# apachepinot/pinot

Measured on AMD Instinct MI355X. Metric: rows scanned/sec, 1B-row segment filter+groupby (3 predicates, SUM/MAX GROUP BY g1), higher is better.
Workload: dtype int64; 1 GPU; 1 segment(s) x 1000000000 rows, one per GPU; SELECT g1, SUM(m), MAX(m) FROM gpuBench WHERE c_inv1 IN (0,1,2,3) AND c_inv2 IN (0,1) AND r_int BETWEEN 250000 AND 749999 GROUP BY g1 ORDER BY g1 LIMIT 1000; query=cfg3, parallelism=segment-per-gpu x1, merge=none (1 segment), entries_scanned_in_filter=249990290

## Files before the change

pinot_amd/csrc/pg_kernels_spec.hip:

```cpp
#define PG_WAVES_PER_BLOCK 12
#define PG_KERNEL template <int PG_NOT_INSTANTIATED> static
#include "pg_kernels.hip"

#define SPEC_LOADERS 4
#ifndef SPEC_TILES
#define SPEC_TILES 2
#endif
#ifndef SPEC_SETS
#define SPEC_SETS 2
#endif
#define SPEC_CONSUMERS 8
#define SPEC_OFF_LIN 0u
#define SPEC_OFF_RNG 256u
#define SPEC_OFF_VAL (256u + 2048u)
#define SPEC_OFF_G0 (256u + 2048u + 8192u)
extern "C" const int pg_spec_waves_per_block = PG_WAVES_PER_BLOCK;
extern "C" int pg_spec_stage_bytes(int bits0, int bits1) { return SPEC_TILES * (((int)SPEC_OFF_G0 + bits0 * 256 + 16 + (bits1 > 0 ? bits1 * 256 + 16 : 0) + 15) & ~15); }

DEVFN void spec_barrier() {
  __builtin_amdgcn_fence(__ATOMIC_RELEASE, "workgroup", "local");
  __builtin_amdgcn_s_barrier();
  __builtin_amdgcn_fence(__ATOMIC_ACQUIRE, "workgroup", "local");
}

template <typename T> DEVFN const GAS T* spec_sgpr_ptr(const void* ptr) {
  const uint64_t v = (uint64_t)ptr;
  const uint32_t lo = (uint32_t)__builtin_amdgcn_readfirstlane((int)(uint32_t)v), hi = (uint32_t)__builtin_amdgcn_readfirstlane((int)(uint32_t)(v >> 32));
  return (const GAS T*)(((uint64_t)hi << 32) | (uint64_t)lo);
}

template <int W> struct SpecCol;
template <> struct SpecCol<0> {};
template <> struct SpecCol<32> { u32x4 r[2]; };
template <> struct SpecCol<24> { u32x4 lo; u32x2 hi; };
template <> struct SpecCol<16> { u32x4 lo; };
template <> struct SpecCol<8> { u32x2 hi; };
constexpr uint32_t spec_img_tile_bytes(int W) { return (uint32_t)(PG_WAVE_DOCS / 8) * (uint32_t)W; }
template <int W> DEVFN void spec_load(SpecCol<W>& c, const uint8_t* base, int wt, int w, int lane) {
  if constexpr (W == 32) {
#pragma unroll
    for (int s = 0; s < 2; s++) {
      const uint8_t* row = base + (size_t)wt * (PG_WAVE_DOCS * 4) + (size_t)(4 * s + w) * 1024u;
      c.r[s] = ldnt((const GAS u32x4*)(spec_sgpr_ptr<uint8_t>(row) + (uint32_t)lane * 16u));
    }
  } else if constexpr (W != 0) {
    const uint8_t* tile = base + (size_t)wt * spec_img_tile_bytes(W);
    if constexpr (W >= 16) c.lo = ldnt((const GAS u32x4*)(spec_sgpr_ptr<uint8_t>(tile + (size_t)w * 1024u) + (uint32_t)lane * 16u));
    if constexpr (W != 16) c.hi = ldnt((const GAS u32x2*)(spec_sgpr_ptr<uint8_t>(tile + (W == 24 ? 4096u : 0u) + (size_t)w * 512u) + (uint32_t)lane * 8u));
  }
}
template <int W> DEVFN void spec_unpack(const SpecCol<W>& c, uint32_t (&a)[4], uint32_t (&b)[4]) {
  if constexpr (W == 32) {
    a[0] = bswap32(c.r[0].x); a[1] = bswap32(c.r[0].y); a[2] = bswap32(c.r[0].z); a[3] = bswap32(c.r[0].w);
    b[0] = bswap32(c.r[1].x); b[1] = bswap32(c.r[1].y); b[2] = bswap32(c.r[1].z); b[3] = bswap32(c.r[1].w);
  } else if constexpr (W == 24) {
    a[0] = __builtin_amdgcn_perm(c.hi.x, c.lo.x, 0x0c040100u); a[1] = __builtin_amdgcn_perm(c.hi.x, c.lo.x, 0x0c050302u);
    a[2] = __builtin_amdgcn_perm(c.hi.x, c.lo.y, 0x0c060100u); a[3] = __builtin_amdgcn_perm(c.hi.x, c.lo.y, 0x0c070302u);
    b[0] = __builtin_amdgcn_perm(c.hi.y, c.lo.z, 0x0c040100u); b[1] = __builtin_amdgcn_perm(c.hi.y, c.lo.z, 0x0c050302u);
    b[2] = __builtin_amdgcn_perm(c.hi.y, c.lo.w, 0x0c060100u); b[3] = __builtin_amdgcn_perm(c.hi.y, c.lo.w, 0x0c070302u);
  } else if constexpr (W == 16) {
    a[0] = c.lo.x & 0xFFFFu; a[1] = c.lo.x >> 16; a[2] = c.lo.y & 0xFFFFu; a[3] = c.lo.y >> 16;
    b[0] = c.lo.z & 0xFFFFu; b[1] = c.lo.z >> 16; b[2] = c.lo.w & 0xFFFFu; b[3] = c.lo.w >> 16;
  } else if constexpr (W == 8) {
#pragma unroll
    for (int e = 0; e < 4; e++) { a[e] = (c.hi.x >> (8 * e)) & 0xFFu; b[e] = (c.hi.y >> (8 * e)) & 0xFFu; }
  }
}
template <int SW, int VW> struct SpecTile {
  SpecCol<SW> scan;
  SpecCol<VW> val;
  u32x4 grp;
};
template <int SW, int VW> struct SpecStage { SpecTile<SW, VW> tile[SPEC_TILES]; uint32_t post[8]; uint32_t tail; };
template <int NG> struct SpecQuad {
  uint32_t lin, rng;
  u32x4 val;
  uint32_t win[NG][2];
};

template <int W> struct SpecWidth { static constexpr int value = W; };
template <int NG, bool HAS_INDEX, bool HAS_SCAN, bool HAS_TAIL = false, bool NARROW = false>
__device__ __forceinline__ void spec_body(const PgQueryPlan& p) {
  extern __shared__ __attribute__((aligned(16))) uint64_t smem[];
  __shared__ uint32_t s_stat[PG_MAX_STATS];
  const int t = threadIdx.x;
  const int lane = t & 63;
  const int wave = uniform(t >> 6);
  int64_t* lds_table = reinterpret_cast<int64_t*>(smem);
  if (t < PG_MAX_STATS) s_stat[t] = 0;
  const uint32_t real_slots = (uint32_t)p.n_groups * (uint32_t)p.replicas;
  const uint32_t table_slots = real_slots + 64u;
  for (int o = 0; o < p.n_ops; o++) {
    const int64_t ident = pg_acc_identity(p.ops[o].fn, p.ops[o].is_float);
    for (uint32_t i = t; i < table_slots; i += PG_BLOCK) lds_table[(size_t)o * table_slots + i] = ident;
  }
  const uint32_t bits0 = (uint32_t)p.gcols[0].bits, bits1 = NG > 1 ? (uint32_t)p.gcols[NG - 1].bits : 0u;
  const uint32_t off_g1 = SPEC_OFF_G0 + bits0 * 256u + 16u;
  const uint32_t tile_bytes = (off_g1 + (NG > 1 ? bits1 * 256u + 16u : 0u) + 15u) & ~15u;
  const uint32_t stage_bytes = tile_bytes * SPEC_TILES;
  uint8_t* stage0 = reinterpret_cast<uint8_t*>(smem) + (((size_t)p.n_ops * table_slots * 8u + 15u) & ~(size_t)15u);
  const CAS PgScanLeaf& L = cptr(p.scans)[HAS_SCAN ? p.fast_scan : 0];
  const int grid = (int)gridDim.x;
  const int n_mine = (int)blockIdx.x < p.n_wtiles ? (p.n_wtiles - (int)blockIdx.x + grid - 1) / grid : 0;
  const int n_stages = (n_mine + SPEC_TILES - 1) / SPEC_TILES;
  __syncthreads();

  if (wave < SPEC_LOADERS) {
    const int w = wave;
    const uint8_t* const xdata = p.srcs[p.pipe_src].data;
    const uint8_t* const simg = NARROW ? p.spec_simg : nullptr;
    const uint8_t* const vimg = NARROW ? p.spec_vimg : nullptr;
    const uint32_t img_slo = NARROW ? p.spec_slo : 0u, img_sspan = NARROW ? p.spec_sspan : 0u, img_vmin = NARROW ? (uint32_t)p.spec_vmin : 0u;
    const bool img_sempty = NARROW && p.spec_sempty != 0;
    const int ggi = (w >> 1) < NG ? (w >> 1) : 0;
    const uint8_t* const gdata = p.gcols[ggi].data;
    const uint32_t gbits = (uint32_t)p.gcols[ggi].bits;
    const uint32_t goff = (uint32_t)(w & 1) * 1024u + (uint32_t)lane * 16u;
    const uint32_t geff = (w >> 1) < NG && goff < gbits * 256u ? goff : 0u;
    const uint8_t* dense_ptr[8];
    int dense_group[8];
#pragma unroll
    for (int j = 0; j < 8; j++) { dense_ptr[j] = HAS_INDEX ? p.dense_ptr[j] : nullptr; dense_group[j] = HAS_INDEX ? p.dense_group[j] : 0; }
    const int dense_groups = p.dense_groups, dense_excl = p.dense_excl;
    const uint8_t* const pipe_tail = HAS_TAIL ? p.pipe_tail : nullptr;
    const int num_docs = p.num_docs;
    const bool scan_pushed = p.fast_scan_pushed != 0;
   auto loaders = [&](auto scan_w, auto val_w) __attribute__((always_inline)) {
    constexpr int SW = HAS_SCAN ? decltype(scan_w)::value : 0, VW = decltype(val_w)::value;
    const RangeI32 r32 = !HAS_SCAN ? RangeI32{0, 0u, false} : (SW == 32 ? make_range_i32(L.lo, L.hi) : RangeI32{(int32_t)img_slo, img_sspan, img_sempty});
    const uint8_t* sdata = !HAS_SCAN ? nullptr : (SW == 32 ? L.data : simg);
    const uint8_t* vdata = VW == 32 ? xdata : vimg;
    const uint32_t vmin = VW == 32 ? 0u : img_vmin;
    uint32_t ld_cand = 0;
    auto issue = [&](int sidx, SpecStage<SW, VW>& st) __attribute__((always_inline)) {
#pragma unroll
      for (int tt = 0; tt < SPEC_TILES; tt++) {
        const int i = sidx * SPEC_TILES + tt;
        const int wt = (int)blockIdx.x + (i < n_mine ? i : n_mine - 1) * grid;
        SpecTile<SW, VW>& tl = st.tile[tt];
        __builtin_amdgcn_sched_barrier(0);
        spec_load<SW>(tl.scan, sdata, wt, w, lane);
        spec_load<VW>(tl.val, vdata, wt, w, lane);
        __builtin_amdgcn_sched_barrier(0);
        {
          const uint8_t* base = gdata + (size_t)wt * (size_t)(PG_WAVE_DOCS / 8) * (size_t)gbits;
          tl.grp = ldnt((const GAS u32x4*)(spec_sgpr_ptr<uint8_t>(base) + geff));
        }
        __builtin_amdgcn_sched_barrier(0);
      }
      if (HAS_INDEX) {
        const int i = sidx * SPEC_TILES + (w % SPEC_TILES);
        const int wt = (int)blockIdx.x + (i < n_mine ? i : n_mine - 1) * grid;
#pragma unroll
        for (int j = 0; j < 8; j++) st.post[j] = *(const GAS uint32_t*)(spec_sgpr_ptr<uint8_t>(dense_ptr[j] + (size_t)wt * 256u) + (uint32_t)lane * 4u);
        __builtin_amdgcn_sched_barrier(0);
      }
      if (HAS_TAIL) {
        const int i = sidx * SPEC_TILES + (w % SPEC_TILES);
        const int wt = (int)blockIdx.x + (i < n_mine ? i : n_mine - 1) * grid;
        st.tail = *(const GAS uint32_t*)(spec_sgpr_ptr<uint8_t>(pipe_tail + (size_t)wt * 256u) + (uint32_t)lane * 4u);
        __builtin_amdgcn_sched_barrier(0);
      }
    };
    auto publish = [&](uint8_t* stage, const SpecStage<SW, VW>& st) __attribute__((always_inline)) {
#ifdef PG_SPEC_NO_PUBLISH
      {
        uint32_t acc = 0;
#pragma unroll
        for (int tt = 0; tt < SPEC_TILES; tt++) {
          uint32_t a[4] = {0u, 0u, 0u, 0u}, b[4] = {0u, 0u, 0u, 0u};
          spec_unpack<SW>(st.tile[tt].scan, a, b); acc += a[0] ^ b[3];
          spec_unpack<VW>(st.tile[tt].val, a, b); acc += a[0] ^ b[3];
          acc += st.tile[tt].grp.x;
        }
        if (acc == 0x12345678u) *reinterpret_cast<uint32_t*>(stage) = acc;
        return;
      }
#endif
#pragma unroll
      for (int tt = 0; tt < SPEC_TILES; tt++) {
        uint8_t* buf = stage + (uint32_t)tt * tile_bytes;
        const SpecTile<SW, VW>& tl = st.tile[tt];
        if (HAS_SCAN) {
          uint32_t q[2][4];
          spec_unpack<SW>(tl.scan, q[0], q[1]);
#pragma unroll
          for (int s = 0; s < 2; s++) {
            uint32_t m = (uint32_t)in_range_i32(r32, (int32_t)q[s][0]) | ((uint32_t)in_range_i32(r32, (int32_t)q[s][1]) << 1) |
                         ((uint32_t)in_range_i32(r32, (int32_t)q[s][2]) << 2) | ((uint32_t)in_range_i32(r32, (int32_t)q[s][3]) << 3);
            m = r32.empty ? 0u : m;
            *reinterpret_cast<uint32_t*>(buf + SPEC_OFF_RNG + (uint32_t)(4 * s + w) * 256u + (uint32_t)lane * 4u) = m;
          }
        }
        {
          uint32_t q[2][4];
          spec_unpack<VW>(tl.val, q[0], q[1]);
#pragma unroll
          for (int s = 0; s < 2; s++) {
            u32x4 v;
            v.x = q[s][0] + vmin; v.y = q[s][1] + vmin; v.z = q[s][2] + vmin; v.w = q[s][3] + vmin;
            *reinterpret_cast<u32x4*>(buf + SPEC_OFF_VAL + (uint32_t)(4 * s + w) * 1024u + (uint32_t)lane * 16u) = v;
          }
        }
        *reinterpret_cast<u32x4*>(buf + (ggi == 0 ? SPEC_OFF_G0 : off_g1) + geff) = tl.grp;
      }
    };
    auto publish_lin = [&](uint8_t* stage, const SpecStage<SW, VW>& st, int sidx) __attribute__((always_inline)) {
      if (w >= SPEC_TILES) return;
      const int i = sidx * SPEC_TILES + w;
      const int wt = (int)blockIdx.x + i * grid;
      const int64_t rem = i < n_mine ? (int64_t)num_docs - (int64_t)wt * PG_WAVE_DOCS : 0;
      const int32_t n_valid = rem >= PG_WAVE_DOCS ? PG_WAVE_DOCS : (rem > 0 ? (int32_t)rem : 0);
      uint32_t lin = valid_lin_mask(n_valid, lane);
      if (HAS_INDEX) {
        uint32_t grp[4] = {0u, 0u, 0u, 0u};
#pragma unroll
        for (int j = 0; j < 8; j++) {
          const int gj = dense_group[j];
#pragma unroll
          for (int k = 0; k < 4; k++) grp[k] |= gj == k ? st.post[j] : 0u;
        }
#pragma unroll
        for (int k = 0; k < 4; k++)
          if (k < dense_groups) lin &= ((dense_excl >> k) & 1) ? ~grp[k] : grp[k];
      }
      *reinterpret_cast<uint32_t*>(stage + (uint32_t)w * tile_bytes + SPEC_OFF_LIN + (uint32_t)lane * 4u) = HAS_TAIL ? lin & st.tail : lin;
      ld_cand += (uint32_t)__popc(lin);
    };
    constexpr int SETS = HAS_SCAN ? SPEC_SETS : 2 * SPEC_SETS;
    SpecStage<SW, VW> st[SETS];
    auto buf_of = [&](int sg) __attribute__((always_inline)) { return stage0 + (uint32_t)(sg & 1) * stage_bytes; };
    if (n_stages > 0) {
#pragma unroll
      for (int k = 0; k < SETS; k++) issue(k, st[k]);
    }
    int s = 0;
    for (; s + SETS - 1 < n_stages; s += SETS) {
#pragma unroll
      for (int k = 0; k < SETS; k++) {
        publish(buf_of(s + k), st[k]);
        publish_lin(buf_of(s + k), st[k], s + k);
        issue(s + k + SETS, st[k]);
        spec_barrier();
      }
    }
#pragma unroll
    for (int k = 0; k < SETS - 1; k++)
      if (s + k < n_stages) {
        publish(buf_of(s + k), st[k]);
        publish_lin(buf_of(s + k), st[k], s + k);
        spec_barrier();
      }
    const uint32_t csum = wave_sum_u32(ld_cand);
    if (HAS_SCAN && !scan_pushed && lane == 0 && csum) atomicAdd(&s_stat[L.stat_slot], csum);
   };
    if constexpr (!NARROW) {
      loaders(SpecWidth<32>{}, SpecWidth<32>{});
    } else {
      const int sb = uniform(p.spec_sbits), vb = uniform(p.spec_vbits);
      auto with_scan = [&](auto scan_w) __attribute__((always_inline)) {
        switch (vb) {
          case 8: loaders(scan_w, SpecWidth<8>{}); break;
          case 16: loaders(scan_w, SpecWidth<16>{}); break;
          case 24: loaders(scan_w, SpecWidth<24>{}); break;
          default: loaders(scan_w, SpecWidth<32>{}); break;
        }
      };
      switch (sb) {
        case 8: with_scan(SpecWidth<8>{}); break;
        case 16: with_scan(SpecWidth<16>{}); break;
        case 24: with_scan(SpecWidth<24>{}); break;
        default: with_scan(SpecWidth<32>{}); break;
      }
    }
  } else {
    const int c = wave - SPEC_LOADERS;
    const uint32_t R = (uint32_t)p.replicas;
    const uint32_t rep = (uint32_t)t & (R - 1u);
    const uint32_t stride = table_slots;
    const uint32_t trash_slot = real_slots + (uint32_t)lane;
    const uint32_t q = (uint32_t)c * 64u + (uint32_t)lane;
    const uint32_t nib = ((uint32_t)lane & 7u) * 4u;
    uint32_t my_matched = 0;
    const int n_ops = uniform(p.n_ops);
    uint64_t ops_code = 0;
    for (int o = 0; o < n_ops; o++) {
      const PgAccOp op = p.ops[uniform(o)];
      ops_code |= (uint64_t)(op.src < 0 ? 0u : (op.fn == PG_ACC_SUM ? 1u : (op.fn == PG_ACC_MIN ? 2u : 3u))) << (2 * o);
    }
    ops_code = ((uint64_t)(uint32_t)uniform((int)(uint32_t)(ops_code >> 32)) << 32) | (uint64_t)(uint32_t)uniform((int)(uint32_t)ops_code);
    const int has_out_words = uniform(p.out_words != nullptr ? 1 : 0);
    auto fetch = [&](const uint8_t* buf, SpecQuad<NG>& d) __attribute__((always_inline)) {
      d.lin = *reinterpret_cast<const uint32_t*>(buf + SPEC_OFF_LIN + (q >> 3) * 4u);
      d.rng = HAS_SCAN ? *reinterpret_cast<const uint32_t*>(buf + SPEC_OFF_RNG + q * 4u) : 0xFu;
      d.val = *reinterpret_cast<const u32x4*>(buf + SPEC_OFF_VAL + q * 16u);
#pragma unroll
      for (int gi = 0; gi < NG; gi++) {
        const uint32_t di = __umul24(4u * q, (uint32_t)p.gcols[gi].bits) >> 5;
        const uint32_t* win = reinterpret_cast<const uint32_t*>(buf + (gi == 0 ? SPEC_OFF_G0 : off_g1)) + di;
        d.win[gi][0] = win[0]; d.win[gi][1] = win[1];
      }
    };
    auto aggregate = [&](const SpecQuad<NG> (&d)[SPEC_TILES], int sidx) __attribute__((always_inline)) {
      constexpr int ND = 4 * SPEC_TILES;
      uint32_t slot[ND];
      int32_t v[ND];
#pragma unroll
      for (int tt = 0; tt < SPEC_TILES; tt++) {
        const int i = sidx * SPEC_TILES + tt;
        const uint32_t cand = (d[tt].lin >> nib) & 0xFu;
        const uint32_t m = d[tt].rng & cand;
        my_matched += (uint32_t)__popc(m);
        if (has_out_words && i < n_mine) {
          const int wt = (int)blockIdx.x + i * grid;
          const uint32_t word = or_reduce8(m << nib);
          if ((lane & 7) == 0) reinterpret_cast<uint32_t*>(p.out_words)[(int64_t)wt * 64 + (int64_t)(q >> 3)] = word;
        }
#ifndef PG_SPEC_NO_TABLE
#pragma unroll
        for (int e = 0; e < 4; e++) slot[4 * tt + e] = rep;
#pragma unroll
        for (int gi = 0; gi < NG; gi++) {
          const PgGroupCol& gc = p.gcols[gi];
          const uint32_t bits = (uint32_t)gc.bits, mask = (1u << gc.bits) - 1u;
          const uint32_t mult = (uint32_t)gc.mult * R;
          uint32_t dv[4];
          decode_packed_quad<true>(d[tt].win[gi], q, bits, mask, dv);
#pragma unroll
          for (int e = 0; e < 4; e++) slot[4 * tt + e] += __umul24(dv[e], mult);
        }
#pragma unroll
        for (int e = 0; e < 4; e++) slot[4 * tt + e] = ((m >> e) & 1u) ? slot[4 * tt + e] : trash_slot;
        v[4 * tt + 0] = (int32_t)d[tt].val.x; v[4 * tt + 1] = (int32_t)d[tt].val.y; v[4 * tt + 2] = (int32_t)d[tt].val.z; v[4 * tt + 3] = (int32_t)d[tt].val.w;
#endif
      }
#ifdef PG_SPEC_NO_TABLE
      return;
#endif
      for (int o = 0; o < n_ops; o++) {
        const uint32_t code = (uint32_t)(ops_code >> (2 * o)) & 3u;
        int64_t* base = lds_table + (size_t)o * stride;
        if (code == 0u) {
#pragma unroll
          for (int e = 0; e < ND; e++) atomicAdd(reinterpret_cast<unsigned long long*>(base + slot[e]), 1ULL);
        } else if (code == 1u) {
#pragma unroll
          for (int e = 0; e < ND; e++) atomicAdd(reinterpret_cast<unsigned long long*>(base + slot[e]), (unsigned long long)(int64_t)v[e]);
        } else if (code == 2u) {
#pragma unroll
          for (int e = 0; e < ND; e++) atomicMin(reinterpret_cast<long long*>(base + slot[e]), (long long)v[e]);
        } else {
#pragma unroll
          for (int e = 0; e < ND; e++) atomicMax(reinterpret_cast<long long*>(base + slot[e]), (long long)v[e]);
        }
      }
    };
    auto fetch_stage = [&](int sidx, SpecQuad<NG> (&d)[SPEC_TILES]) __attribute__((always_inline)) {
// ... 83 lines not shown
```

pinot_amd/csrc/pg_segment.cpp:

```cpp
#include <hip/hip_runtime.h>

#include <algorithm>
#include <cmath>

#include "pg_internal.hpp"

extern "C" __global__ void __launch_bounds__(256) pg_column_magnitude_kernel(const uint8_t* __restrict__ data, int64_t n, int val_type,
                                                                             unsigned long long* __restrict__ out) {
  unsigned long long mx = 0, bad = 0;
  for (int64_t i = (int64_t)blockIdx.x * blockDim.x + threadIdx.x; i < n; i += (int64_t)gridDim.x * blockDim.x) {
    unsigned long long a;
    if (val_type == PG_V_I64) {
      const unsigned long long v = __builtin_bswap64(reinterpret_cast<const unsigned long long*>(data)[i]);
      a = (long long)v < 0 ? 0ULL - v : v;
    } else {
      double d;
      if (val_type == PG_V_F32) d = (double)__uint_as_float(__builtin_bswap32(reinterpret_cast<const uint32_t*>(data)[i]));
      else d = __longlong_as_double((long long)__builtin_bswap64(reinterpret_cast<const unsigned long long*>(data)[i]));
      a = (unsigned long long)__double_as_longlong(d) & 0x7FFFFFFFFFFFFFFFULL;
      if (a >= 0x7FF0000000000000ULL) { bad = 1; a = 0; }
    }
    mx = a > mx ? a : mx;
  }
  for (int off = 32; off > 0; off >>= 1) {
    const unsigned long long o = __shfl_xor(mx, off, 64);
    mx = o > mx ? o : mx;
    bad |= __shfl_xor(bad, off, 64);
  }
  if ((threadIdx.x & 63) == 0) {
    if (mx) atomicMax(&out[0], mx);
    if (bad) atomicOr(&out[1], 1ULL);
  }
}

extern "C" __global__ void __launch_bounds__(256) pg_column_int_range_kernel(const uint8_t* __restrict__ data, int64_t n, int val_type,
                                                                             long long* __restrict__ out) {
  long long mn = INT64_MAX, mx = INT64_MIN;
  for (int64_t i = (int64_t)blockIdx.x * blockDim.x + threadIdx.x; i < n; i += (int64_t)gridDim.x * blockDim.x) {
    const long long v = val_type == PG_V_I64 ? (long long)__builtin_bswap64(reinterpret_cast<const unsigned long long*>(data)[i])
                                             : (long long)(int32_t)__builtin_bswap32(reinterpret_cast<const uint32_t*>(data)[i]);
    mn = v < mn ? v : mn;
    mx = v > mx ? v : mx;
  }
  for (int off = 32; off > 0; off >>= 1) {
    const long long a = __shfl_xor(mn, off, 64), b = __shfl_xor(mx, off, 64);
    mn = a < mn ? a : mn;
    mx = b > mx ? b : mx;
  }
  if ((threadIdx.x & 63) == 0 && mn <= mx) {
    atomicMin(&out[0], mn);
    atomicMax(&out[1], mx);
  }
}

extern "C" __global__ void __launch_bounds__(256) pg_column_narrow_image_kernel(const uint8_t* __restrict__ data, uint8_t* __restrict__ img,
                                                                                int64_t n_wtiles, int32_t vmin, int bits) {
  const int64_t n = n_wtiles * 256;
  const int64_t tile_bytes = (int64_t)(PG_WAVE_DOCS / 8) * bits;
  for (int64_t i = (int64_t)blockIdx.x * blockDim.x + threadIdx.x; i < n; i += (int64_t)gridDim.x * blockDim.x) {
    const int64_t wt = i >> 8;
    const int b = (int)(i >> 6) & 3, l = (int)i & 63;
    const uint4 qa = *reinterpret_cast<const uint4*>(data + wt * (PG_WAVE_DOCS * 4) + (int64_t)b * 1024 + l * 16);
    const uint4 qb = *reinterpret_cast<const uint4*>(data + wt * (PG_WAVE_DOCS * 4) + (int64_t)(4 + b) * 1024 + l * 16);
    const uint32_t raw[8] = {qa.x, qa.y, qa.z, qa.w, qb.x, qb.y, qb.z, qb.w};
    uint32_t s[8];
    for (int e = 0; e < 8; e++) s[e] = (__builtin_bswap32(raw[e]) - (uint32_t)vmin) & (bits == 24 ? 0xFFFFFFu : (bits == 16 ? 0xFFFFu : 0xFFu));
    uint8_t* tile = img + wt * tile_bytes;
    if (bits >= 16) {
      uint4 lo;
      lo.x = (s[0] & 0xFFFFu) | (s[1] << 16); lo.y = (s[2] & 0xFFFFu) | (s[3] << 16);
      lo.z = (s[4] & 0xFFFFu) | (s[5] << 16); lo.w = (s[6] & 0xFFFFu) | (s[7] << 16);
      *reinterpret_cast<uint4*>(tile + (int64_t)b * 1024 + l * 16) = lo;
    }
    if (bits != 16) {
      const int sh = bits == 24 ? 16 : 0;
      uint2 hi;
      hi.x = ((s[0] >> sh) & 0xFFu) | (((s[1] >> sh) & 0xFFu) << 8) | (((s[2] >> sh) & 0xFFu) << 16) | (((s[3] >> sh) & 0xFFu) << 24);
      hi.y = ((s[4] >> sh) & 0xFFu) | (((s[5] >> sh) & 0xFFu) << 8) | (((s[6] >> sh) & 0xFFu) << 16) | (((s[7] >> sh) & 0xFFu) << 24);
      *reinterpret_cast<uint2*>(tile + (bits == 24 ? 4096 : 0) + (int64_t)b * 512 + l * 8) = hi;
    }
  }
}

extern "C" __global__ void __launch_bounds__(256) pg_column_max_dict_id_kernel(const uint8_t* __restrict__ data, int64_t n, int bits,
                                                                                unsigned int* __restrict__ out) {
  unsigned int mx = 0;
  const uint64_t mask = (1ULL << bits) - 1ULL;
  for (int64_t i = (int64_t)blockIdx.x * blockDim.x + threadIdx.x; i < n; i += (int64_t)gridDim.x * blockDim.x) {
    const uint64_t bit = (uint64_t)i * (uint64_t)bits;
    const uint8_t* p = data + (bit >> 3);
    uint64_t w = 0;
    for (int k = 0; k < 8; k++) w = (w << 8) | p[k];
    const unsigned int v = (unsigned int)((w >> (64 - bits - (int)(bit & 7))) & mask);
    mx = v > mx ? v : mx;
  }
  for (int off = 32; off > 0; off >>= 1) {
    const unsigned int o = __shfl_xor(mx, off, 64);
    mx = o > mx ? o : mx;
  }
  if ((threadIdx.x & 63) == 0 && mx) atomicMax(out, mx);
}

namespace pg {

static int32_t fx_exp_of(double max_abs) {
  if (!(max_abs > 0)) return 0;
  int e = 0;
  (void)std::frexp(max_abs, &e);
  return (int32_t)(16 * (int)std::floor(((double)e + 15.0) / 16.0));
}

static inline uint32_t be32(const uint8_t* p) {
  return ((uint32_t)p[0] << 24) | ((uint32_t)p[1] << 16) | ((uint32_t)p[2] << 8) | (uint32_t)p[3];
}
static inline uint64_t be64(const uint8_t* p) { return ((uint64_t)be32(p) << 32) | be32(p + 4); }
static inline uint16_t le16(const uint8_t* p) { return (uint16_t)(p[0] | (p[1] << 8)); }
static inline uint32_t le32(const uint8_t* p) {
  return (uint32_t)p[0] | ((uint32_t)p[1] << 8) | ((uint32_t)p[2] << 16) | ((uint32_t)p[3] << 24);
}

Column* Segment::find(const char* n) {
  if (!n) return nullptr;
  auto it = columns.find(n);
  return it == columns.end() ? nullptr : it->second.get();
}

static size_t padded_docs(const Segment& seg) { return (size_t)seg.n_tiles * PG_TILE_DOCS; }

static void check_dict_ids(const Column& c, int64_t n) {
  if (n <= 0 || c.cardinality <= 0 || !(c.bits >= 31 || ((int64_t)1 << c.bits) > (int64_t)c.cardinality)) return;
  DeviceBuffer out(4, true);
  const int grid = (int)std::max<int64_t>(1, std::min<int64_t>(2048, (n + 255) / 256));
  hipLaunchKernelGGL(pg_column_max_dict_id_kernel, dim3(grid), dim3(256), 0, 0, c.fwd_dev.as<uint8_t>(), n, c.bits, out.as<unsigned int>());
  PG_HIP(hipGetLastError());
  unsigned int mx = 0;
  PG_HIP(hipMemcpy(&mx, out.ptr, 4, hipMemcpyDeviceToHost));
  if ((int64_t)mx >= (int64_t)c.cardinality)
    fail(PG_ERR_INVALID_ARGUMENT, "forward index of %s holds dictId %u, the dictionary has %d values", c.name.c_str(), mx, c.cardinality);
}

static void upload_fixed_bit(Segment& seg, Column& c, const uint8_t* src, uint64_t len) {
  uint64_t need = ((uint64_t)seg.total_docs * (uint64_t)c.bits + 7) / 8;
  if (len < need) fail(PG_ERR_INVALID_ARGUMENT, "forward index of %s is %llu bytes, need %llu", c.name.c_str(),
                       (unsigned long long)len, (unsigned long long)need);
  size_t alloc = (padded_docs(seg) * (size_t)c.bits + 7) / 8 + 64;
  c.fwd_dev.alloc(alloc, true);
  c.fwd_dev.upload(src, need);
  c.col_kind = PG_COL_FIXED_BIT;
  c.fwd_bytes_logical = need;
  check_dict_ids(c, (int64_t)seg.total_docs);
}

static void parse_inverted_index(Segment& seg, Column& c, const uint8_t* inv, uint64_t len) {
  const int32_t card = c.cardinality;
  const uint64_t off_end = ((uint64_t)card + 1) * 4;
  if (len < off_end) fail(PG_ERR_INVALID_ARGUMENT, "inverted index of %s too short", c.name.c_str());
  const uint64_t first = be32(inv);
  const uint8_t* bitmap_buffer = inv + off_end;
  c.posting_begin.assign((size_t)card + 1, 0);
  std::vector<uint8_t> staging;
  staging.reserve(len);
  const uint32_t max_key = (uint32_t)((padded_docs(seg) + PG_CHUNK_DOCS - 1) / PG_CHUNK_DOCS);
// ... 693 lines not shown
      offs.resize((size_t)used_chunks + 1);
      decompress_fixed_byte_chunks(compression, fwd, offs, (uint32_t)docs_per_chunk * (uint32_t)width, need, c.fwd_dev.as<uint8_t>(), d.name);
    }
    c.col_kind = width == 4 ? PG_COL_RAW32 : PG_COL_RAW64;
    c.fwd_bytes_logical = need;
  } else {
    fail(PG_ERR_UNSUPPORTED, "column %s: forward index encoding %d", d.name, c.fwd_encoding);
  }

  if (c.has_dictionary && (c.data_type == PG_TYPE_LONG || c.data_type == PG_TYPE_FLOAT || c.data_type == PG_TYPE_DOUBLE)) {
    const uint8_t* dp = c.dict_host.data();
    double mx = 0;
    for (int32_t i = 0; i < c.cardinality; i++) {
      if (c.data_type == PG_TYPE_LONG) {
        const int64_t v = (int64_t)be64(dp + (size_t)i * 8);
        const uint64_t a = v < 0 ? 0ULL - (uint64_t)v : (uint64_t)v;
        c.max_abs_int = std::max(c.max_abs_int, a);
      } else {
        double v;
        if (c.data_type == PG_TYPE_FLOAT) { uint32_t u = be32(dp + (size_t)i * 4); float f; memcpy(&f, &u, 4); v = (double)f; }
        else { uint64_t u = be64(dp + (size_t)i * 8); memcpy(&v, &u, 8); }
        if (std::isfinite(v)) mx = std::max(mx, std::fabs(v));
        else c.has_nonfinite = true;
      }
    }
    c.fx_exp = fx_exp_of(mx);
  } else if (!c.has_dictionary && (c.val_type == PG_V_I64 || c.val_type == PG_V_F32 || c.val_type == PG_V_F64) &&
             (c.col_kind == PG_COL_RAW32 || c.col_kind == PG_COL_RAW64) && seg.total_docs > 0) {
    DeviceBuffer out(16, true);
    hipLaunchKernelGGL(pg_column_magnitude_kernel, dim3(1024), dim3(256), 0, 0, c.fwd_dev.as<uint8_t>(), (int64_t)seg.total_docs, c.val_type,
                       out.as<unsigned long long>());
    PG_HIP(hipGetLastError());
    unsigned long long h[2] = {0, 0};
    PG_HIP(hipMemcpy(h, out.ptr, sizeof(h), hipMemcpyDeviceToHost));
    if (c.val_type == PG_V_I64) c.max_abs_int = h[0];
    else {
      double mx;
      memcpy(&mx, &h[0], 8);
      c.fx_exp = fx_exp_of(mx);
      c.has_nonfinite = h[1] != 0;
    }
  }

  if (!c.has_dictionary && (c.val_type == PG_V_I32 || c.val_type == PG_V_I64) && (c.col_kind == PG_COL_RAW32 || c.col_kind == PG_COL_RAW64) &&
      seg.total_docs > 0) {
    const long long init[2] = {INT64_MAX, INT64_MIN};
    DeviceBuffer out(16);
    out.upload(init, sizeof(init));
    hipLaunchKernelGGL(pg_column_int_range_kernel, dim3(1024), dim3(256), 0, 0, c.fwd_dev.as<uint8_t>(), (int64_t)seg.total_docs, c.val_type,
                       out.as<long long>());
    PG_HIP(hipGetLastError());
    long long h[2] = {0, 0};
    PG_HIP(hipMemcpy(h, out.ptr, sizeof(h), hipMemcpyDeviceToHost));
    if (h[0] <= h[1]) { c.has_int_range = true; c.int_min = h[0]; c.int_max = h[1]; }
  }

  if (d.inverted_index.size > 0 && c.has_dictionary && c.fwd_encoding != PG_FWD_DICT_SORTED)
    parse_inverted_index(seg, c, (const uint8_t*)d.inverted_index.addr, d.inverted_index.size);

  seg.device_bytes += c.fwd_dev.size + c.dict_dev.size + c.containers_dev.size + c.descs_dev.size + c.mv_offsets_dev.size + c.vb_offsets_dev.size;
  seg.columns.emplace(c.name, std::move(col));
}

bool narrow_image_eligible(const Column& c) {
  return !c.has_dictionary && !c.is_mv && !c.raw_mv && c.col_kind == PG_COL_RAW32 && c.val_type == PG_V_I32 && c.has_int_range &&
         c.int_max - c.int_min < ((int64_t)1 << 24);
}

bool narrow_image(Segment& seg, Column& c) {
  std::lock_guard<std::mutex> g(seg.mu);
  if (c.img_state != 0) return c.img_state == 1;
  c.img_state = 2;
  const int64_t n_wtiles = (int64_t)seg.n_tiles * PG_WTILES_PER_TILE;
  if (!narrow_image_eligible(c) || n_wtiles <= 0 || c.fwd_dev.size < (size_t)n_wtiles * (PG_WAVE_DOCS * 4)) return false;
  const int64_t span = c.int_max - c.int_min;
  const int bits = span < 256 ? 8 : (span < 65536 ? 16 : 24);
  void* ptr = nullptr;
  const size_t bytes = (size_t)(n_wtiles * narrow_image_tile_bytes(bits));
  if (hipMalloc(&ptr, bytes) != hipSuccess) {
    (void)hipGetLastError();
    return false;
  }
  c.img_dev.ptr = ptr; c.img_dev.size = bytes; c.img_dev.device = seg.device;
  const int grid = (int)std::min<int64_t>((n_wtiles * 256 + 255) / 256, 8192);
  hipLaunchKernelGGL(pg_column_narrow_image_kernel, dim3(grid), dim3(256), 0, 0, c.fwd_dev.as<uint8_t>(), c.img_dev.as<uint8_t>(), n_wtiles,
                     (int32_t)c.int_min, bits);
  PG_HIP(hipGetLastError());
  PG_HIP(hipDeviceSynchronize());
  c.img_bits = bits;
  c.img_state = 1;
  seg.device_bytes += bytes;
  return true;
}

}
```

Baseline: 820.7 billion rows/s.

## Assign each spec loader wave a half-tile with wider loads and split roles

Loader waves change from loading a quarter-row slice of both tiles in a stage to owning one half of a single tile (tile w>>1, half w&1). Each wave now issues wider contiguous loads: four 16-byte rows for 32-bit data, and 16-byte instead of 8-byte high-byte loads for narrow data. It also loads every group column itself, and only the half-0 waves fetch the index postings and tail. The narrow-image layout and the kernel that builds it are rearranged to match the per-half contiguous layout. The aim is fewer, larger, better-coalesced memory requests and less per-wave work on postings. The cost is more registers per wave and a doubled template instantiation through the role parameter.

```diff
diff --git a/pinot_amd/csrc/pg_kernels_spec.hip b/pinot_amd/csrc/pg_kernels_spec.hip
--- a/pinot_amd/csrc/pg_kernels_spec.hip
+++ b/pinot_amd/csrc/pg_kernels_spec.hip
@@ -31,47 +31,56 @@
 
 template <int W> struct SpecCol;
 template <> struct SpecCol<0> {};
-template <> struct SpecCol<32> { u32x4 r[2]; };
-template <> struct SpecCol<24> { u32x4 lo; u32x2 hi; };
-template <> struct SpecCol<16> { u32x4 lo; };
-template <> struct SpecCol<8> { u32x2 hi; };
+template <> struct SpecCol<32> { u32x4 r[4]; };
+template <> struct SpecCol<24> { u32x4 lo[2]; u32x4 hi; };
+template <> struct SpecCol<16> { u32x4 lo[2]; };
+template <> struct SpecCol<8> { u32x4 hi; };
 constexpr uint32_t spec_img_tile_bytes(int W) { return (uint32_t)(PG_WAVE_DOCS / 8) * (uint32_t)W; }
-template <int W> DEVFN void spec_load(SpecCol<W>& c, const uint8_t* base, int wt, int w, int lane) {
+template <int W> DEVFN void spec_load(SpecCol<W>& c, const uint8_t* base, int wt, int h, int lane) {
   if constexpr (W == 32) {
 #pragma unroll
-    for (int s = 0; s < 2; s++) {
-      const uint8_t* row = base + (size_t)wt * (PG_WAVE_DOCS * 4) + (size_t)(4 * s + w) * 1024u;
-      c.r[s] = ldnt((const GAS u32x4*)(spec_sgpr_ptr<uint8_t>(row) + (uint32_t)lane * 16u));
+    for (int r = 0; r < 4; r++) {
+      const uint8_t* row = base + (size_t)wt * (PG_WAVE_DOCS * 4) + (size_t)(4 * h + r) * 1024u;
+      c.r[r] = ldnt((const GAS u32x4*)(spec_sgpr_ptr<uint8_t>(row) + (uint32_t)lane * 16u));
     }
   } else if constexpr (W != 0) {
-    const uint8_t* tile = base + (size_t)wt * spec_img_tile_bytes(W);
-    if constexpr (W >= 16) c.lo = ldnt((const GAS u32x4*)(spec_sgpr_ptr<uint8_t>(tile + (size_t)w * 1024u) + (uint32_t)lane * 16u));
-    if constexpr (W != 16) c.hi = ldnt((const GAS u32x2*)(spec_sgpr_ptr<uint8_t>(tile + (W == 24 ? 4096u : 0u) + (size_t)w * 512u) + (uint32_t)lane * 8u));
-  }
-}
-template <int W> DEVFN void spec_unpack(const SpecCol<W>& c, uint32_t (&a)[4], uint32_t (&b)[4]) {
+    const uint8_t* half = base + (size_t)wt * spec_img_tile_bytes(W) + (size_t)h * (spec_img_tile_bytes(W) / 2u);
+    if constexpr (W >= 16) {
+#pragma unroll
+      for (int r = 0; r < 2; r++) c.lo[r] = ldnt((const GAS u32x4*)(spec_sgpr_ptr<uint8_t>(half + (size_t)r * 1024u) + (uint32_t)lane * 16u));
+    }
+    if constexpr (W != 16) c.hi = ldnt((const GAS u32x4*)(spec_sgpr_ptr<uint8_t>(half + (W == 24 ? 2048u : 0u)) + (uint32_t)lane * 16u));
+  }
+}
+template <int W> DEVFN void spec_unpack(const SpecCol<W>& c, uint32_t (&q)[4][4]) {
   if constexpr (W == 32) {
-    a[0] = bswap32(c.r[0].x); a[1] = bswap32(c.r[0].y); a[2] = bswap32(c.r[0].z); a[3] = bswap32(c.r[0].w);
-    b[0] = bswap32(c.r[1].x); b[1] = bswap32(c.r[1].y); b[2] = bswap32(c.r[1].z); b[3] = bswap32(c.r[1].w);
-  } else if constexpr (W == 24) {
-    a[0] = __builtin_amdgcn_perm(c.hi.x, c.lo.x, 0x0c040100u); a[1] = __builtin_amdgcn_perm(c.hi.x, c.lo.x, 0x0c050302u);
-    a[2] = __builtin_amdgcn_perm(c.hi.x, c.lo.y, 0x0c060100u); a[3] = __builtin_amdgcn_perm(c.hi.x, c.lo.y, 0x0c070302u);
-    b[0] = __builtin_amdgcn_perm(c.hi.y, c.lo.z, 0x0c040100u); b[1] = __builtin_amdgcn_perm(c.hi.y, c.lo.z, 0x0c050302u);
-    b[2] = __builtin_amdgcn_perm(c.hi.y, c.lo.w, 0x0c060100u); b[3] = __builtin_amdgcn_perm(c.hi.y, c.lo.w, 0x0c070302u);
-  } else if constexpr (W == 16) {
-    a[0] = c.lo.x & 0xFFFFu; a[1] = c.lo.x >> 16; a[2] = c.lo.y & 0xFFFFu; a[3] = c.lo.y >> 16;
-    b[0] = c.lo.z & 0xFFFFu; b[1] = c.lo.z >> 16; b[2] = c.lo.w & 0xFFFFu; b[3] = c.lo.w >> 16;
+#pragma unroll
+    for (int r = 0; r < 4; r++) { q[r][0] = bswap32(c.r[r].x); q[r][1] = bswap32(c.r[r].y); q[r][2] = bswap32(c.r[r].z); q[r][3] = bswap32(c.r[r].w); }
+  } else if constexpr (W == 24 || W == 16) {
+    const uint32_t lw[8] = {c.lo[0].x, c.lo[0].y, c.lo[0].z, c.lo[0].w, c.lo[1].x, c.lo[1].y, c.lo[1].z, c.lo[1].w};
+    if constexpr (W == 24) {
+      const uint32_t hw[4] = {c.hi.x, c.hi.y, c.hi.z, c.hi.w};
+#pragma unroll
+      for (int r = 0; r < 4; r++) {
+        q[r][0] = __builtin_amdgcn_perm(hw[r], lw[2 * r], 0x0c040100u); q[r][1] = __builtin_amdgcn_perm(hw[r], lw[2 * r], 0x0c050302u);
+        q[r][2] = __builtin_amdgcn_perm(hw[r], lw[2 * r + 1], 0x0c060100u); q[r][3] = __builtin_amdgcn_perm(hw[r], lw[2 * r + 1], 0x0c070302u);
+      }
+    } else {
+#pragma unroll
+      for (int r = 0; r < 4; r++) { q[r][0] = lw[2 * r] & 0xFFFFu; q[r][1] = lw[2 * r] >> 16; q[r][2] = lw[2 * r + 1] & 0xFFFFu; q[r][3] = lw[2 * r + 1] >> 16; }
+    }
   } else if constexpr (W == 8) {
-#pragma unroll
-    for (int e = 0; e < 4; e++) { a[e] = (c.hi.x >> (8 * e)) & 0xFFu; b[e] = (c.hi.y >> (8 * e)) & 0xFFu; }
-  }
-}
-template <int SW, int VW> struct SpecTile {
-  SpecCol<SW> scan;
-  SpecCol<VW> val;
-  u32x4 grp;
-};
-template <int SW, int VW> struct SpecStage { SpecTile<SW, VW> tile[SPEC_TILES]; uint32_t post[8]; uint32_t tail; };
+    const uint32_t hw[4] = {c.hi.x, c.hi.y, c.hi.z, c.hi.w};
+#pragma unroll
+    for (int r = 0; r < 4; r++)
+#pragma unroll
+      for (int e = 0; e < 4; e++) q[r][e] = (hw[r] >> (8 * e)) & 0xFFu;
+  }
+}
+template <bool LIN> struct SpecPost;
+template <> struct SpecPost<true> { uint32_t post[8]; uint32_t tail; };
+template <> struct SpecPost<false> {};
+template <int SW, int VW, int NG, bool LIN> struct SpecStage { SpecCol<SW> scan; SpecCol<VW> val; u32x4 grp[NG]; SpecPost<LIN> ix; };
 template <int NG> struct SpecQuad {
   uint32_t lin, rng;
   u32x4 val;
@@ -79,6 +88,7 @@
 };
 
 template <int W> struct SpecWidth { static constexpr int value = W; };
+template <bool LIN> struct SpecRole { static constexpr bool value = LIN; };
 template <int NG, bool HAS_INDEX, bool HAS_SCAN, bool HAS_TAIL = false, bool NARROW = false>
 __device__ __forceinline__ void spec_body(const PgQueryPlan& p) {
   extern __shared__ __attribute__((aligned(16))) uint64_t smem[];
@@ -107,16 +117,22 @@
 
   if (wave < SPEC_LOADERS) {
     const int w = wave;
+    static_assert(SPEC_TILES == 2 && SPEC_LOADERS == 4, "loader w owns half w & 1 of tile w >> 1 of a stage");
+    const int T = w >> 1, h = w & 1;
     const uint8_t* const xdata = p.srcs[p.pipe_src].data;
     const uint8_t* const simg = NARROW ? p.spec_simg : nullptr;
     const uint8_t* const vimg = NARROW ? p.spec_vimg : nullptr;
     const uint32_t img_slo = NARROW ? p.spec_slo : 0u, img_sspan = NARROW ? p.spec_sspan : 0u, img_vmin = NARROW ? (uint32_t)p.spec_vmin : 0u;
     const bool img_sempty = NARROW && p.spec_sempty != 0;
-    const int ggi = (w >> 1) < NG ? (w >> 1) : 0;
-    const uint8_t* const gdata = p.gcols[ggi].data;
-    const uint32_t gbits = (uint32_t)p.gcols[ggi].bits;
-    const uint32_t goff = (uint32_t)(w & 1) * 1024u + (uint32_t)lane * 16u;
-    const uint32_t geff = (w >> 1) < NG && goff < gbits * 256u ? goff : 0u;
+    const uint8_t* gdata[NG];
+    uint32_t gbits[NG], geff[NG];
+#pragma unroll
+    for (int gi = 0; gi < NG; gi++) {
+      gdata[gi] = p.gcols[gi].data;
+      gbits[gi] = (uint32_t)p.gcols[gi].bits;
+      const uint32_t goff = (uint32_t)h * 1024u + (uint32_t)lane * 16u;
+      geff[gi] = goff < gbits[gi] * 256u ? goff : 0u;
+    }
     const uint8_t* dense_ptr[8];
     int dense_group[8];
 #pragma unroll
@@ -125,110 +141,101 @@
     const uint8_t* const pipe_tail = HAS_TAIL ? p.pipe_tail : nullptr;
     const int num_docs = p.num_docs;
     const bool scan_pushed = p.fast_scan_pushed != 0;
-   auto loaders = [&](auto scan_w, auto val_w) __attribute__((always_inline)) {
+   auto loaders = [&](auto scan_w, auto val_w, auto role) __attribute__((always_inline)) {
     constexpr int SW = HAS_SCAN ? decltype(scan_w)::value : 0, VW = decltype(val_w)::value;
+    constexpr bool LIN = decltype(role)::value;
+    using Stage = SpecStage<SW, VW, NG, LIN>;
     const RangeI32 r32 = !HAS_SCAN ? RangeI32{0, 0u, false} : (SW == 32 ? make_range_i32(L.lo, L.hi) : RangeI32{(int32_t)img_slo, img_sspan, img_sempty});
     const uint8_t* sdata = !HAS_SCAN ? nullptr : (SW == 32 ? L.data : simg);
     const uint8_t* vdata = VW == 32 ? xdata : vimg;
     const uint32_t vmin = VW == 32 ? 0u : img_vmin;
     uint32_t ld_cand = 0;
-    auto issue = [&](int sidx, SpecStage<SW, VW>& st) __attribute__((always_inline)) {
-#pragma unroll
-      for (int tt = 0; tt < SPEC_TILES; tt++) {
-        const int i = sidx * SPEC_TILES + tt;
-        const int wt = (int)blockIdx.x + (i < n_mine ? i : n_mine - 1) * grid;
-        SpecTile<SW, VW>& tl = st.tile[tt];
+    auto issue = [&](int sidx, Stage& st) __attribute__((always_inline)) {
+      const int i = sidx * SPEC_TILES + T;
+      const int wt = (int)blockIdx.x + (i < n_mine ? i : n_mine - 1) * grid;
+      __builtin_amdgcn_sched_barrier(0);
+      spec_load<SW>(st.scan, sdata, wt, h, lane);
+      spec_load<VW>(st.val, vdata, wt, h, lane);
+      __builtin_amdgcn_sched_barrier(0);
+#pragma unroll
+      for (int gi = 0; gi < NG; gi++) {
+        const uint8_t* base = gdata[gi] + (size_t)wt * (size_t)(PG_WAVE_DOCS / 8) * (size_t)gbits[gi];
+        st.grp[gi] = ldnt((const GAS u32x4*)(spec_sgpr_ptr<uint8_t>(base) + geff[gi]));
         __builtin_amdgcn_sched_barrier(0);
-        spec_load<SW>(tl.scan, sdata, wt, w, lane);
-        spec_load<VW>(tl.val, vdata, wt, w, lane);
+      }
+      if constexpr (LIN && HAS_INDEX) {
+#pragma unroll
+        for (int j = 0; j < 8; j++) st.ix.post[j] = *(const GAS uint32_t*)(spec_sgpr_ptr<uint8_t>(dense_ptr[j] + (size_t)wt * 256u) + (uint32_t)lane * 4u);
         __builtin_amdgcn_sched_barrier(0);
-        {
-          const uint8_t* base = gdata + (size_t)wt * (size_t)(PG_WAVE_DOCS / 8) * (size_t)gbits;
-          tl.grp = ldnt((const GAS u32x4*)(spec_sgpr_ptr<uint8_t>(base) + geff));
-        }
+      }
+      if constexpr (LIN && HAS_TAIL) {
+        st.ix.tail = *(const GAS uint32_t*)(spec_sgpr_ptr<uint8_t>(pipe_tail + (size_t)wt * 256u) + (uint32_t)lane * 4u);
         __builtin_amdgcn_sched_barrier(0);
       }
-      if (HAS_INDEX) {
-        const int i = sidx * SPEC_TILES + (w % SPEC_TILES);
-        const int wt = (int)blockIdx.x + (i < n_mine ? i : n_mine - 1) * grid;
-#pragma unroll
-        for (int j = 0; j < 8; j++) st.post[j] = *(const GAS uint32_t*)(spec_sgpr_ptr<uint8_t>(dense_ptr[j] + (size_t)wt * 256u) + (uint32_t)lane * 4u);
-        __builtin_amdgcn_sched_barrier(0);
-      }
-      if (HAS_TAIL) {
-        const int i = sidx * SPEC_TILES + (w % SPEC_TILES);
-        const int wt = (int)blockIdx.x + (i < n_mine ? i : n_mine - 1) * grid;
-        st.tail = *(const GAS uint32_t*)(spec_sgpr_ptr<uint8_t>(pipe_tail + (size_t)wt * 256u) + (uint32_t)lane * 4u);
-        __builtin_amdgcn_sched_barrier(0);
-      }
-    };
-    auto publish = [&](uint8_t* stage, const SpecStage<SW, VW>& st) __attribute__((always_inline)) {
+    };
+    auto publish = [&](uint8_t* stage, const Stage& st) __attribute__((always_inline)) {
 #ifdef PG_SPEC_NO_PUBLISH
       {
         uint32_t acc = 0;
-#pragma unroll
-        for (int tt = 0; tt < SPEC_TILES; tt++) {
-          uint32_t a[4] = {0u, 0u, 0u, 0u}, b[4] = {0u, 0u, 0u, 0u};
-          spec_unpack<SW>(st.tile[tt].scan, a, b); acc += a[0] ^ b[3];
-          spec_unpack<VW>(st.tile[tt].val, a, b); acc += a[0] ^ b[3];
-          acc += st.tile[tt].grp.x;
-        }
+        uint32_t q[4][4] = {};
+        spec_unpack<SW>(st.scan, q); acc += q[0][0] ^ q[3][3];
+        spec_unpack<VW>(st.val, q); acc += q[0][0] ^ q[3][3];
+#pragma unroll
+        for (int gi = 0; gi < NG; gi++) acc += st.grp[gi].x;
         if (acc == 0x12345678u) *reinterpret_cast<uint32_t*>(stage) = acc;
         return;
       }
 #endif
-#pragma unroll
-      for (int tt = 0; tt < SPEC_TILES; tt++) {
-        uint8_t* buf = stage + (uint32_t)tt * tile_bytes;
-        const SpecTile<SW, VW>& tl = st.tile[tt];
-        if (HAS_SCAN) {
-          uint32_t q[2][4];
-          spec_unpack<SW>(tl.scan, q[0], q[1]);
-#pragma unroll
-          for (int s = 0; s < 2; s++) {
-            uint32_t m = (uint32_t)in_range_i32(r32, (int32_t)q[s][0]) | ((uint32_t)in_range_i32(r32, (int32_t)q[s][1]) << 1) |
-                         ((uint32_t)in_range_i32(r32, (int32_t)q[s][2]) << 2) | ((uint32_t)in_range_i32(r32, (int32_t)q[s][3]) << 3);
-            m = r32.empty ? 0u : m;
-            *reinterpret_cast<uint32_t*>(buf + SPEC_OFF_RNG + (uint32_t)(4 * s + w) * 256u + (uint32_t)lane * 4u) = m;
+      uint8_t* buf = stage + (uint32_t)T * tile_bytes;
+      if (HAS_SCAN) {
+        uint32_t q[4][4];
+        spec_unpack<SW>(st.scan, q);
+#pragma unroll
+        for (int r = 0; r < 4; r++) {
+          uint32_t m = (uint32_t)in_range_i32(r32, (int32_t)q[r][0]) | ((uint32_t)in_range_i32(r32, (int32_t)q[r][1]) << 1) |
+                       ((uint32_t)in_range_i32(r32, (int32_t)q[r][2]) << 2) | ((uint32_t)in_range_i32(r32, (int32_t)q[r][3]) << 3);
+          m = r32.empty ? 0u : m;
+          *reinterpret_cast<uint32_t*>(buf + SPEC_OFF_RNG + (uint32_t)(4 * h + r) * 256u + (uint32_t)lane * 4u) = m;
+        }
+      }
+      {
+        uint32_t q[4][4];
+        spec_unpack<VW>(st.val, q);
+#pragma unroll
+        for (int r = 0; r < 4; r++) {
+          u32x4 v;
+          v.x = q[r][0] + vmin; v.y = q[r][1] + vmin; v.z = q[r][2] + vmin; v.w = q[r][3] + vmin;
+          *reinterpret_cast<u32x4*>(buf + SPEC_OFF_VAL + (uint32_t)(4 * h + r) * 1024u + (uint32_t)lane * 16u) = v;
+        }
+      }
+#pragma unroll
+      for (int gi = 0; gi < NG; gi++) *reinterpret_cast<u32x4*>(buf + (gi == 0 ? SPEC_OFF_G0 : off_g1) + geff[gi]) = st.grp[gi];
+    };
+    auto publish_lin = [&](uint8_t* stage, const Stage& st, int sidx) __attribute__((always_inline)) {
+      if constexpr (LIN) {
+        const int i = sidx * SPEC_TILES + T;
+        const int wt = (int)blockIdx.x + i * grid;
+        const int64_t rem = i < n_mine ? (int64_t)num_docs - (int64_t)wt * PG_WAVE_DOCS : 0;
+        const int32_t n_valid = rem >= PG_WAVE_DOCS ? PG_WAVE_DOCS : (rem > 0 ? (int32_t)rem : 0);
+        uint32_t lin = valid_lin_mask(n_valid, lane);
+        if (HAS_INDEX) {
+          uint32_t grp[4] = {0u, 0u, 0u, 0u};
+#pragma unroll
+          for (int j = 0; j < 8; j++) {
+            const int gj = dense_group[j];
+#pragma unroll
+            for (int k = 0; k < 4; k++) grp[k] |= gj == k ? st.ix.post[j] : 0u;
           }
-        }
-        {
-          uint32_t q[2][4];
-          spec_unpack<VW>(tl.val, q[0], q[1]);
-#pragma unroll
-          for (int s = 0; s < 2; s++) {
-            u32x4 v;
-            v.x = q[s][0] + vmin; v.y = q[s][1] + vmin; v.z = q[s][2] + vmin; v.w = q[s][3] + vmin;
-            *reinterpret_cast<u32x4*>(buf + SPEC_OFF_VAL + (uint32_t)(4 * s + w) * 1024u + (uint32_t)lane * 16u) = v;
-          }
-        }
-        *reinterpret_cast<u32x4*>(buf + (ggi == 0 ? SPEC_OFF_G0 : off_g1) + geff) = tl.grp;
-      }
-    };
-    auto publish_lin = [&](uint8_t* stage, const SpecStage<SW, VW>& st, int sidx) __attribute__((always_inline)) {
-      if (w >= SPEC_TILES) return;
-      const int i = sidx * SPEC_TILES + w;
-      const int wt = (int)blockIdx.x + i * grid;
-      const int64_t rem = i < n_mine ? (int64_t)num_docs - (int64_t)wt * PG_WAVE_DOCS : 0;
-      const int32_t n_valid = rem >= PG_WAVE_DOCS ? PG_WAVE_DOCS : (rem > 0 ? (int32_t)rem : 0);
-      uint32_t lin = valid_lin_mask(n_valid, lane);
-      if (HAS_INDEX) {
-        uint32_t grp[4] = {0u, 0u, 0u, 0u};
-#pragma unroll
-        for (int j = 0; j < 8; j++) {
-          const int gj = dense_group[j];
-#pragma unroll
-          for (int k = 0; k < 4; k++) grp[k] |= gj == k ? st.post[j] : 0u;
-        }
-#pragma unroll
-        for (int k = 0; k < 4; k++)
-          if (k < dense_groups) lin &= ((dense_excl >> k) & 1) ? ~grp[k] : grp[k];
-      }
-      *reinterpret_cast<uint32_t*>(stage + (uint32_t)w * tile_bytes + SPEC_OFF_LIN + (uint32_t)lane * 4u) = HAS_TAIL ? lin & st.tail : lin;
-      ld_cand += (uint32_t)__popc(lin);
+#pragma unroll
+          for (int k = 0; k < 4; k++)
+            if (k < dense_groups) lin &= ((dense_excl >> k) & 1) ? ~grp[k] : grp[k];
+        }
+        *reinterpret_cast<uint32_t*>(stage + (uint32_t)T * tile_bytes + SPEC_OFF_LIN + (uint32_t)lane * 4u) = HAS_TAIL ? lin & st.ix.tail : lin;
+        ld_cand += (uint32_t)__popc(lin);
+      }
     };
     constexpr int SETS = HAS_SCAN ? SPEC_SETS : 2 * SPEC_SETS;
-    SpecStage<SW, VW> st[SETS];
+    Stage st[SETS];
     auto buf_of = [&](int sg) __attribute__((always_inline)) { return stage0 + (uint32_t)(sg & 1) * stage_bytes; };
     if (n_stages > 0) {
 #pragma unroll
@@ -254,25 +261,29 @@
     const uint32_t csum = wave_sum_u32(ld_cand);
     if (HAS_SCAN && !scan_pushed && lane == 0 && csum) atomicAdd(&s_stat[L.stat_slot], csum);
    };
-    if constexpr (!NARROW) {
-      loaders(SpecWidth<32>{}, SpecWidth<32>{});
-    } else {
-      const int sb = uniform(p.spec_sbits), vb = uniform(p.spec_vbits);
-      auto with_scan = [&](auto scan_w) __attribute__((always_inline)) {
-        switch (vb) {
-          case 8: loaders(scan_w, SpecWidth<8>{}); break;
-          case 16: loaders(scan_w, SpecWidth<16>{}); break;
-          case 24: loaders(scan_w, SpecWidth<24>{}); break;
-          default: loaders(scan_w, SpecWidth<32>{}); break;
-        }
-      };
-      switch (sb) {
-        case 8: with_scan(SpecWidth<8>{}); break;
-        case 16: with_scan(SpecWidth<16>{}); break;
-        case 24: with_scan(SpecWidth<24>{}); break;
-        default: with_scan(SpecWidth<32>{}); break;
-      }
-    }
+    auto with_role = [&](auto role) __attribute__((always_inline)) {
+      if constexpr (!NARROW) {
+        loaders(SpecWidth<32>{}, SpecWidth<32>{}, role);
+      } else {
+        const int sb = uniform(p.spec_sbits), vb = uniform(p.spec_vbits);
+        auto with_scan = [&](auto scan_w) __attribute__((always_inline)) {
+          switch (vb) {
+            case 8: loaders(scan_w, SpecWidth<8>{}, role); break;
+            case 16: loaders(scan_w, SpecWidth<16>{}, role); break;
+            case 24: loaders(scan_w, SpecWidth<24>{}, role); break;
+            default: loaders(scan_w, SpecWidth<32>{}, role); break;
+          }
+        };
+        switch (sb) {
+          case 8: with_scan(SpecWidth<8>{}); break;
+          case 16: with_scan(SpecWidth<16>{}); break;
+          case 24: with_scan(SpecWidth<24>{}); break;
+          default: with_scan(SpecWidth<32>{}); break;
+        }
+      }
+    };
+    if (h == 0) with_role(SpecRole<true>{});
+    else with_role(SpecRole<false>{});
   } else {
     const int c = wave - SPEC_LOADERS;
     const uint32_t R = (uint32_t)p.replicas;
diff --git a/pinot_amd/csrc/pg_segment.cpp b/pinot_amd/csrc/pg_segment.cpp
--- a/pinot_amd/csrc/pg_segment.cpp
+++ b/pinot_amd/csrc/pg_segment.cpp
@@ -55,29 +55,39 @@
 
 extern "C" __global__ void __launch_bounds__(256) pg_column_narrow_image_kernel(const uint8_t* __restrict__ data, uint8_t* __restrict__ img,
                                                                                 int64_t n_wtiles, int32_t vmin, int bits) {
-  const int64_t n = n_wtiles * 256;
+  const int64_t n = n_wtiles * 128;
   const int64_t tile_bytes = (int64_t)(PG_WAVE_DOCS / 8) * bits;
   for (int64_t i = (int64_t)blockIdx.x * blockDim.x + threadIdx.x; i < n; i += (int64_t)gridDim.x * blockDim.x) {
-    const int64_t wt = i >> 8;
-    const int b = (int)(i >> 6) & 3, l = (int)i & 63;
-    const uint4 qa = *reinterpret_cast<const uint4*>(data + wt * (PG_WAVE_DOCS * 4) + (int64_t)b * 1024 + l * 16);
-    const uint4 qb = *reinterpret_cast<const uint4*>(data + wt * (PG_WAVE_DOCS * 4) + (int64_t)(4 + b) * 1024 + l * 16);
-    const uint32_t raw[8] = {qa.x, qa.y, qa.z, qa.w, qb.x, qb.y, qb.z, qb.w};
-    uint32_t s[8];
-    for (int e = 0; e < 8; e++) s[e] = (__builtin_bswap32(raw[e]) - (uint32_t)vmin) & (bits == 24 ? 0xFFFFFFu : (bits == 16 ? 0xFFFFu : 0xFFu));
-    uint8_t* tile = img + wt * tile_bytes;
+    const int64_t wt = i >> 7;
+    const int h = (int)(i >> 6) & 1, l = (int)i & 63;
+    uint32_t s[16];
+#pragma unroll
+    for (int r = 0; r < 4; r++) {
+      const uint4 q = *reinterpret_cast<const uint4*>(data + wt * (PG_WAVE_DOCS * 4) + (int64_t)(4 * h + r) * 1024 + l * 16);
+      const uint32_t raw[4] = {q.x, q.y, q.z, q.w};
+#pragma unroll
+      for (int e = 0; e < 4; e++) s[4 * r + e] = (__builtin_bswap32(raw[e]) - (uint32_t)vmin) & (bits == 24 ? 0xFFFFFFu : (bits == 16 ? 0xFFFFu : 0xFFu));
+    }
+    uint8_t* half = img + wt * tile_bytes + (int64_t)h * (tile_bytes / 2);
     if (bits >= 16) {
-      uint4 lo;
-      lo.x = (s[0] & 0xFFFFu) | (s[1] << 16); lo.y = (s[2] & 0xFFFFu) | (s[3] << 16);
-      lo.z = (s[4] & 0xFFFFu) | (s[5] << 16); lo.w = (s[6] & 0xFFFFu) | (s[7] << 16);
-      *reinterpret_cast<uint4*>(tile + (int64_t)b * 1024 + l * 16) = lo;
+#pragma unroll
+      for (int r = 0; r < 2; r++) {
+        const uint32_t* d = s + 8 * r;
+        uint4 lo;
+        lo.x = (d[0] & 0xFFFFu) | (d[1] << 16); lo.y = (d[2] & 0xFFFFu) | (d[3] << 16);
+        lo.z = (d[4] & 0xFFFFu) | (d[5] << 16); lo.w = (d[6] & 0xFFFFu) | (d[7] << 16);
+        *reinterpret_cast<uint4*>(half + (int64_t)r * 1024 + l * 16) = lo;
+      }
     }
     if (bits != 16) {
       const int sh = bits == 24 ? 16 : 0;
-      uint2 hi;
-      hi.x = ((s[0] >> sh) & 0xFFu) | (((s[1] >> sh) & 0xFFu) << 8) | (((s[2] >> sh) & 0xFFu) << 16) | (((s[3] >> sh) & 0xFFu) << 24);
-      hi.y = ((s[4] >> sh) & 0xFFu) | (((s[5] >> sh) & 0xFFu) << 8) | (((s[6] >> sh) & 0xFFu) << 16) | (((s[7] >> sh) & 0xFFu) << 24);
-      *reinterpret_cast<uint2*>(tile + (bits == 24 ? 4096 : 0) + (int64_t)b * 512 + l * 8) = hi;
+      uint32_t hw[4];
+#pragma unroll
+      for (int r = 0; r < 4; r++) {
+        const uint32_t* d = s + 4 * r;
+        hw[r] = ((d[0] >> sh) & 0xFFu) | (((d[1] >> sh) & 0xFFu) << 8) | (((d[2] >> sh) & 0xFFu) << 16) | (((d[3] >> sh) & 0xFFu) << 24);
+      }
+      *reinterpret_cast<uint4*>(half + (bits == 24 ? 2048 : 0) + l * 16) = make_uint4(hw[0], hw[1], hw[2], hw[3]);
     }
   }
 }
@@ -937,7 +947,7 @@
     return false;
   }
   c.img_dev.ptr = ptr; c.img_dev.size = bytes; c.img_dev.device = seg.device;
-  const int grid = (int)std::min<int64_t>((n_wtiles * 256 + 255) / 256, 8192);
+  const int grid = (int)std::min<int64_t>((n_wtiles * 128 + 255) / 256, 8192);
   hipLaunchKernelGGL(pg_column_narrow_image_kernel, dim3(grid), dim3(256), 0, 0, c.fwd_dev.as<uint8_t>(), c.img_dev.as<uint8_t>(), n_wtiles,
                      (int32_t)c.int_min, bits);
   PG_HIP(hipGetLastError());
```

Result: no change. 827.4 billion rows/s, median of 6 (+0.8%).
